# erlgo/openair4G

Measured on AMD Instinct MI355X. Metric: DL subframes/sec (20 MHz, 2x2, 64-QAM), higher is better.
Workload: dtype int16; 1 GPU; dlsim 20 MHz 2x2 TM3 (LARGE_CDD) 64-QAM MCS19x2CW, 2x14 IDFT-2048; config_id=C3, global_batch=8192, subframe_index=7, full_grid=False, parallelism=subframe-sharded x1

## Files before the change

include/oai4g.h:

```cpp
#ifndef OAI4G_H
#define OAI4G_H

#include <stddef.h>
#include <stdint.h>

#ifdef __cplusplus
extern "C" {
#endif

#define OAI4G_LTE_NULL 2
#define OAI4G_NSOFT 1827072
#define OAI4G_MAX_SEGMENTS 16
#define OAI4G_MAX_CHANNEL_BITS (14 * 1200 * 6)
#define OAI4G_D_BYTES (96 + 12 + 3 + 3 * 6144)
#define OAI4G_W_BYTES (3 * 6144 + 96)

enum { OAI4G_SISO = 0, OAI4G_ALAMOUTI = 1, OAI4G_LARGE_CDD = 2 };
enum { OAI4G_CYCLIC_PREFIX = 0, OAI4G_CYCLIC_SUFFIX = 1, OAI4G_ZEROS = 2, OAI4G_NONE = 3 };

typedef struct {
  uint16_t N_RB_DL;
  uint16_t Nid_cell;
  uint8_t Ncp;
  uint8_t nushift;
// ... 57 lines not shown

int oai4g_init(void);
const char *oai4g_last_error(void);
int oai4g_device_name(char *buf, int len);

int oai4g_init_frame_parms(oai4g_frame_parms_t *fp, uint16_t N_RB_DL, uint16_t Nid_cell, uint8_t Ncp,
                           uint8_t nb_antennas_tx, uint8_t mode1_flag, uint8_t frame_type);
uint8_t oai4g_get_Qm(uint8_t mcs);
int oai4g_get_G(const oai4g_frame_parms_t *fp, uint16_t nb_rb, const uint32_t *rb_alloc, uint8_t mod_order,
                uint8_t Nl, uint8_t num_pdcch_symbols, int frame, uint8_t subframe);
uint8_t oai4g_get_Qm_ul(uint8_t mcs);
uint8_t oai4g_get_I_TBS(uint8_t mcs);
uint8_t oai4g_get_I_TBS_UL(uint8_t mcs);
uint32_t oai4g_tbs_bits(uint8_t I_TBS, uint16_t nb_rb);
uint32_t oai4g_get_TBS_DL(uint8_t mcs, uint16_t nb_rb);
uint32_t oai4g_get_TBS_UL(uint8_t mcs, uint16_t nb_rb);
oai4g_dlsch_t *oai4g_new_dlsch(uint8_t Kmimo, uint8_t Mdlharq, uint8_t N_RB_DL);
void oai4g_free_dlsch(oai4g_dlsch_t *dlsch);
uint32_t oai4g_lte_gold_generic(uint32_t *x1, uint32_t *x2, uint8_t reset);
int oai4g_qpp_fold32(uint32_t K, uint32_t *s, uint16_t *tab);
int oai4g_rsc_scan_rows(uint32_t q, uint32_t rows[6]);
int oai4g_rm_pair_schedule(uint32_t C, uint32_t n0, const uint32_t nt[2], const uint32_t wrapt[2],
                           uint32_t *pairs, uint32_t *pair0);

uint32_t oai4g_crc24a(const uint8_t *in, int bitlen);
uint32_t oai4g_crc24b(const uint8_t *in, int bitlen);
int oai4g_lte_segmentation(const uint8_t *input_buffer, uint8_t **output_buffers, uint32_t B, uint32_t *C,
                           uint32_t *Cplus, uint32_t *Cminus, uint32_t *Kplus, uint32_t *Kminus, uint32_t *F);
void oai4g_threegpplte_turbo_encoder(const uint8_t *input, uint16_t input_length_bytes, uint8_t *output,
                                     uint8_t F, uint16_t interleaver_f1, uint16_t interleaver_f2);
uint32_t oai4g_sub_block_interleaving_turbo(uint32_t D, uint8_t *d, uint8_t *w);
uint32_t oai4g_lte_rate_matching_turbo(uint32_t RTC, uint32_t G, const uint8_t *w, uint8_t *e, uint8_t C,
                                       uint32_t Nsoft, uint8_t Mdlharq, uint8_t Kmimo, uint8_t rvidx,
                                       uint8_t Qm, uint8_t Nl, uint8_t r, uint8_t nb_rb, uint8_t m);
int oai4g_dlsch_encoding(uint8_t *a, const oai4g_frame_parms_t *frame_parms, uint8_t num_pdcch_symbols,
                         oai4g_dlsch_t *dlsch, int frame, uint8_t subframe);
void oai4g_dlsch_scrambling(const oai4g_frame_parms_t *frame_parms, int mbsfn_flag, oai4g_dlsch_t *dlsch, int G,
                            uint8_t q, uint8_t Ns);
int oai4g_dlsch_modulation(int32_t **txdataF, int16_t amp, uint32_t subframe_offset,
                           const oai4g_frame_parms_t *frame_parms, uint8_t num_pdcch_symbols,
                           oai4g_dlsch_t *dlsch0, oai4g_dlsch_t *dlsch1);
void oai4g_PHY_ofdm_mod(const int32_t *input, int32_t *output, uint8_t log2fftsize, uint8_t nb_symbols,
                        uint16_t nb_prefix_samples, int etype);
void oai4g_normal_prefix_mod(const int32_t *txdataF, int32_t *txdata, uint8_t nsymb,
                             const oai4g_frame_parms_t *frame_parms);
void oai4g_do_OFDM_mod(int32_t **txdataF, int32_t **txdata, uint32_t frame, uint16_t next_slot,
// ... 208 lines not shown

int oai4g_tx_batch(const oai4g_tx_config_t *cfg, int n_sf, const uint8_t *d_payload, void *d_work,
                   int32_t *d_iq, void *stream);
int oai4g_tx_batch_timed(const oai4g_tx_config_t *cfg, int n_sf, const uint8_t *d_payload, void *d_work,
                         int32_t *d_iq, void *stream, float *kernel_ms);
int oai4g_tx_config_set_control(oai4g_tx_config_t *cfg, uint8_t num_ue_spec_dci, uint8_t num_common_dci,
                                const oai4g_dci_alloc_t *dci_alloc);
#define OAI4G_MAX_PHICH_ITEMS 64
typedef struct {
  uint8_t subframe, ngroup, nseq, hi;
} oai4g_phich_item_t;
typedef struct {
  uint8_t pss_sss;
  uint8_t pbch;
  uint8_t pbch_pdu[3];
  uint8_t frame_mod4;
  uint8_t n_phich;
  oai4g_phich_item_t phich[OAI4G_MAX_PHICH_ITEMS];
} oai4g_common_sig_t;
int oai4g_tx_config_set_common(oai4g_tx_config_t *cfg, const oai4g_common_sig_t *common);
int oai4g_tx_encode(const oai4g_tx_config_t *cfg, int n_sf, const uint8_t *d_payload, void *d_work, void *stream);
int oai4g_tx_modulate(const oai4g_tx_config_t *cfg, int n_sf, const void *d_work, int32_t *d_iq, void *stream);
int oai4g_tx_mod_nosat(const oai4g_tx_config_t *cfg);

int oai4g_diag_encode_phase_ms(const oai4g_tx_config_t *cfg, int n_sf, const uint8_t *d_payload, void *d_work,
                               int stop_phase, int reps, float *ms);
int oai4g_diag_encode_occupancy(const oai4g_tx_config_t *cfg, int *blocks_per_cu, size_t *lds_bytes);
int oai4g_diag_stream(const void *d_src, void *d_dst, size_t bytes, int mode, void *stream);

int oai4g_set_device(int device);
#define OAI4G_DIST_ID_BYTES 128
int oai4g_dist_unique_id(uint8_t id[OAI4G_DIST_ID_BYTES]);
int oai4g_dist_init(int rank, int world, const uint8_t id[OAI4G_DIST_ID_BYTES]);
int oai4g_dist_broadcast_params(oai4g_tx_params_t *p, int root);
int oai4g_dist_allreduce_sum_u64(uint64_t *v, int n);
int oai4g_dist_allreduce_max_f64(double *v, int n);
int oai4g_dist_barrier(void);
int oai4g_dist_rank(void);
int oai4g_dist_world(void);
int oai4g_dist_finalize(void);
void oai4g_shard_range(int n_total, int rank, int world, int *first, int *count);
uint64_t oai4g_payload_seed(uint64_t seed, uint64_t first_subframe, uint32_t n_cw, uint32_t payload_stride);

void *oai4g_dev_alloc(size_t bytes);
void oai4g_dev_free(void *p);
int oai4g_memcpy_h2d(void *dst, const void *src, size_t bytes);
// ... 10 lines not shown
```

openair4g_amd/__init__.py:

```python
import ctypes
import os

import numpy as np

_HERE = os.path.dirname(os.path.abspath(__file__))
LIB_PATH = os.path.join(_HERE, "lib", "libopenair4g_amd.so")

LTE_NULL = 2
NSOFT = 1827072
MAX_SEGMENTS = 16
MAX_CHANNEL_BITS = 14 * 1200 * 6
D_BYTES = 96 + 12 + 3 + 3 * 6144
W_BYTES = 3 * 6144 + 96
SISO, ALAMOUTI, LARGE_CDD = 0, 1, 2
CYCLIC_PREFIX = 0


class OAI4GError(RuntimeError):
    pass


u8p = ctypes.POINTER(ctypes.c_uint8)


# ... 278 lines not shown
    "oai4g_tx_encode": (ctypes.c_int, [ctypes.c_void_p, ctypes.c_int, ctypes.c_void_p, ctypes.c_void_p,
                                       ctypes.c_void_p]),
    "oai4g_tx_modulate": (ctypes.c_int, [ctypes.c_void_p, ctypes.c_int, ctypes.c_void_p, ctypes.c_void_p,
                                         ctypes.c_void_p]),
    "oai4g_tx_mod_nosat": (ctypes.c_int, [ctypes.c_void_p]),
    "oai4g_diag_encode_phase_ms": (ctypes.c_int, [ctypes.c_void_p, ctypes.c_int, ctypes.c_void_p, ctypes.c_void_p,
                                                  ctypes.c_int, ctypes.c_int, ctypes.POINTER(ctypes.c_float)]),
    "oai4g_diag_encode_occupancy": (ctypes.c_int, [ctypes.c_void_p, ctypes.POINTER(ctypes.c_int),
                                                   ctypes.POINTER(ctypes.c_size_t)]),
    "oai4g_diag_stream": (ctypes.c_int, [ctypes.c_void_p, ctypes.c_void_p, ctypes.c_size_t, ctypes.c_int,
                                         ctypes.c_void_p]),
    "oai4g_dev_alloc": (ctypes.c_void_p, [ctypes.c_size_t]),
    "oai4g_dev_free": (None, [ctypes.c_void_p]),
    "oai4g_memcpy_h2d": (ctypes.c_int, [ctypes.c_void_p, ctypes.c_void_p, ctypes.c_size_t]),
    "oai4g_memcpy_d2h": (ctypes.c_int, [ctypes.c_void_p, ctypes.c_void_p, ctypes.c_size_t]),
    "oai4g_memset_d": (ctypes.c_int, [ctypes.c_void_p, ctypes.c_int, ctypes.c_size_t]),
    "oai4g_sync": (ctypes.c_int, []),
    "oai4g_fill_payload": (ctypes.c_int, [ctypes.c_void_p, ctypes.c_size_t, ctypes.c_uint64, ctypes.c_void_p]),
    "oai4g_qpp_fold32": (ctypes.c_int, [ctypes.c_uint32, ctypes.POINTER(ctypes.c_uint32), ctypes.c_void_p]),
    "oai4g_rsc_scan_rows": (ctypes.c_int, [ctypes.c_uint32, ctypes.POINTER(ctypes.c_uint32)]),
    "oai4g_rm_pair_schedule": (ctypes.c_int, [ctypes.c_uint32, ctypes.c_uint32, ctypes.POINTER(ctypes.c_uint32),
                                              ctypes.POINTER(ctypes.c_uint32), ctypes.POINTER(ctypes.c_uint32),
                                              ctypes.POINTER(ctypes.c_uint32)]),
}


def load_library(path=None):
    global _lib
    if _lib is not None:
        return _lib
    path = path or os.environ.get("OAI4G_LIB") or LIB_PATH
    if not os.path.exists(path):
        raise OAI4GError(f"HIP library not built: {path} (run __graft_entry__.build())")
    lib = ctypes.CDLL(path)
    for name, (res, args) in _SIGS.items():
        fn = getattr(lib, name)
        fn.restype = res
        fn.argtypes = args
    _lib = lib
    return lib


def exported_symbols():
    return sorted(_SIGS)


# ... 979 lines not shown
        return ms[0], ms[1]

    def encode_only(self, stream=None):
        _check(self.L.oai4g_tx_encode(self.cfg, self.n_sf, self.d_payload, self.d_work, stream) == 0)

    def diag_encode_phase_ms(self, stop_phase, reps=5):
        ms = ctypes.c_float()
        _check(self.L.oai4g_diag_encode_phase_ms(self.cfg, self.n_sf, self.d_payload, self.d_work, stop_phase, reps,
                                                 ctypes.byref(ms)) == 0)
        return ms.value

    def modulate_only(self, stream=None):
        _check(self.L.oai4g_tx_modulate(self.cfg, self.n_sf, self.d_work, self.d_iq, stream) == 0)

    def upload_ebits(self, words):
        words = np.ascontiguousarray(words, dtype=np.uint32)
        assert words.nbytes <= self.work_bytes
        _check(self.L.oai4g_memcpy_h2d(self.d_work, _ptr(words), words.nbytes) == 0)

    @property
    def mod_nosat(self):
        return bool(self.L.oai4g_tx_mod_nosat(self.cfg))

    def sync(self):
        _check(self.L.oai4g_sync() == 0)

    def ebits(self):
        out = np.empty(self.work_bytes // 4, dtype=np.uint32)
        _check(self.L.oai4g_memcpy_d2h(_ptr(out), self.d_work, out.nbytes) == 0)
        return out.reshape(self.n_sf, self.n_cw, self.ebits_words)

    def iq(self):
        out = np.empty(self.iq_samples, dtype=np.int32)
        _check(self.L.oai4g_memcpy_d2h(_ptr(out), self.d_iq, out.nbytes) == 0)
        return out.reshape(self.n_sf, self.n_ant, self.spt)

    def close(self):
        for p in (self.d_payload, self.d_work, self.d_iq):
            if p:
                self.L.oai4g_dev_free(p)
        self.d_payload = self.d_work = self.d_iq = None
        if self.cfg:
            self.L.oai4g_tx_config_destroy(self.cfg)
            self.cfg = None

    def __del__(self):
# ... 10 lines not shown
```

openair4g_amd/csrc/oai4g_host.cpp:

```cpp
#include <hip/hip_runtime.h>
#include <math.h>
#include <pthread.h>
#include <stdarg.h>
#include <stdio.h>
#include <stdlib.h>
#include <string.h>

#include <algorithm>
#include <cmath>
#include <cstdlib>
#include <vector>
#include <map>
#include <mutex>
#include <vector>

#include "../../include/oai4g.h"
#include "../../include/oai4g_qpp.h"
#include "../../include/oai4g_tbs.h"
#include "oai4g_internal.h"

static thread_local char g_err[512] = "";

static void set_err(const char *fmt, ...)
{
// ... 486 lines not shown
static uint32_t mod_nosat_ok(const cfg_dev_t &h, int v_static)
{
  if (h.log2N != 11 || h.nsymb != 14 || getenv("OAI4G_MOD_SAT")) return 0;
  int v = v_static;
  for (uint32_t cw = 0; cw < h.n_cw; cw++) {
    const cw_dev_t &c = h.cw[cw];
    for (int i = 0; i < 8; i++) v = std::max(v, std::max(std::abs((int)c.qam_a[i]), std::abs((int)c.qam_b[i])));
    v = std::max(v, std::max(std::abs((int)c.qpsk_a), std::abs((int)c.qpsk_b)));
    for (int i = 0; i < 2; i++)
      v = std::max(v, std::max(std::abs((int)c.alm_qpsk[i][0]), std::abs((int)c.alm_qpsk[i][1])));
  }
  const double R = std::sqrt(2.0) * v, band = 12.0 * h.N_RB_DL;
  const double c32 = std::ceil(band / 32) + 1, c8 = std::ceil(band / 8) + 1, c2 = std::ceil(band / 2) + 1;
  return (c32 * R + 128 <= 32767 && c8 * R / 8 + 128 <= 32767 && c2 * R / 16 + 128 <= 32767 &&
          (band + 1) * R / 32 + 128 <= 32767) ? 1u : 0u;
}

static int packed_iq_max(const std::vector<uint32_t> &t)
{
  int v = 0;
  for (uint32_t w : t) v = std::max(v, std::max(std::abs((int)(int16_t)(w & 0xFFFFu)), std::abs((int)(int16_t)(w >> 16))));
  return v;
}

static int not_pilot(int pilots, int re, int nushift, int use2nd)
{
  int off = (pilots == 2) ? 3 : 0, v = nushift % 3;
  if (pilots == 0) return 1;
  if (use2nd) return (re != nushift + off) && (re != ((nushift + 6 + off) % 12));
  return (re != v) && (re != v + 6) && (re != v + 3) && (re != v + 9);
}

static int build_remap(const oai4g_frame_parms_t *fp, const uint32_t *rb_alloc, int num_pdcch, int subframe,
                       int mimo_mode, uint16_t *remap , uint32_t *symbase ,
                       int *re_alloc )
{
  const bool alm = mimo_mode == OAI4G_ALAMOUTI;
  int ralloc = 0;
  int N = fp->ofdm_symbol_size, nsymb = fp->Ncp == 0 ? 14 : 12, half = fp->N_RB_DL >> 1;
  int use2nd = fp->mode1_flag == 1;
  for (int i = 0; i < 14 * N; i++) remap[i] = 0xFFFF;
  uint32_t total = 0;
  for (int l = 0; l < 14; l++) symbase[l] = 0;
  for (int l = num_pdcch; l < nsymb; l++) {
    symbase[l] = total;
    uint32_t idx = 0;
// ... 620 lines not shown
      };
      for (int n = 1; n < 50; n++) step();
      const size_t nw = std::min(stride, (size_t)(h.cw[cw].G[sf] + 31) / 32);
      uint32_t *o = g.data() + ((size_t)sf * h.n_cw + cw) * stride;
      for (size_t w = 0; w < nw; w++) {
        step();
        o[w] = x1 ^ x2;
      }
    }
  if (cfg->d_gold) hipFree(cfg->d_gold);
  cfg->d_gold = nullptr;
  HCK(hipMalloc(&cfg->d_gold, g.size() * 4), -1);
  HCK(hipMemcpy(cfg->d_gold, g.data(), g.size() * 4, hipMemcpyHostToDevice), -1);
  cfg->h.gold_tab = cfg->d_gold;
  return 0;
}

static int upload_cfg(oai4g_tx_config *cfg)
{
  if (upload_remap(cfg) != 0) return -1;
  if (upload_gold(cfg) != 0) return -1;
  cfg->h.with_crs = !cfg->h_crs.empty();
  cfg->h.mod_nosat = mod_nosat_ok(cfg->h, std::max(packed_iq_max(cfg->h_crs), cfg->ctl_vmax));
  cfg->h.n_cu = (uint32_t)g_n_cu;
  cfg->h.gold_x1 = g_gx1;
  cfg->h.gold_x2j = g_gx2j;
  cfg->h.tw = g_tw;
  HCK(hipMalloc(&cfg->d, sizeof(cfg_dev_t)), -1);
  HCK(hipMemcpy(cfg->d, &cfg->h, sizeof(cfg_dev_t), hipMemcpyHostToDevice), -1);
  return 0;
}

static void release_cfg(oai4g_tx_config *cfg)
{
  for (auto &e : cfg->ev_enc)
    if (e) hipEventDestroy(e);
  if (cfg->ev_done) hipEventDestroy(cfg->ev_done);
  if (cfg->s_mod) hipStreamDestroy(cfg->s_mod);
  cfg->s_mod = nullptr;
  cfg->ev_done = nullptr;
  if (cfg->d) hipFree(cfg->d);
  if (cfg->d_remap) hipFree(cfg->d_remap);
  if (cfg->d_stat) hipFree(cfg->d_stat);
  if (cfg->d_gold) hipFree(cfg->d_gold);
  cfg->d_stat = nullptr;
  cfg->d_gold = nullptr;
// ... 106 lines not shown
  for (int i = 0; i < 3; i++) HCK(hipEventCreate(&ev[i]), -1);
  HCK(hipEventRecord(ev[0], s), -1);
  HCK(oai4g_launch_encode(cfg->d, &cfg->h, 0, n_sf, d_payload, (uint32_t *)d_work, s), -1);
  HCK(hipEventRecord(ev[1], s), -1);
  HCK(oai4g_launch_modofdm(cfg->d, &cfg->h, 0, n_sf, (const uint32_t *)d_work, d_iq, s), -1);
  HCK(hipEventRecord(ev[2], s), -1);
  HCK(hipEventSynchronize(ev[2]), -1);
  HCK(hipEventElapsedTime(&kernel_ms[0], ev[0], ev[1]), -1);
  HCK(hipEventElapsedTime(&kernel_ms[1], ev[1], ev[2]), -1);
  for (int i = 0; i < 3; i++) hipEventDestroy(ev[i]);
  return 0;
}

extern "C" int oai4g_tx_modulate(const oai4g_tx_config_t *cfg, int n_sf, const void *d_work, int32_t *d_iq,
                                 void *stream)
{
  NEED_INIT(-1);
  if (!cfg || !iq_aligned(d_iq)) return -1;
  HCK(oai4g_launch_modofdm(cfg->d, &cfg->h, 0, n_sf, (const uint32_t *)d_work, d_iq, (hipStream_t)stream), -1);
  return 0;
}

extern "C" int oai4g_tx_mod_nosat(const oai4g_tx_config_t *cfg) { return cfg ? (int)cfg->h.mod_nosat : 0; }

extern "C" int oai4g_diag_encode_phase_ms(const oai4g_tx_config_t *cfg, int n_sf, const uint8_t *d_payload,
                                          void *d_work, int stop_phase, int reps, float *ms)
{
  NEED_INIT(-1);
  hipEvent_t a, b;
  HCK(hipEventCreate(&a), -1);
  HCK(hipEventCreate(&b), -1);
  HCK(oai4g_launch_encode_phase(cfg->d, &cfg->h, n_sf, d_payload, (uint32_t *)d_work, stop_phase, nullptr), -1);
  HCK(hipEventRecord(a, nullptr), -1);
  for (int i = 0; i < reps; i++)
    HCK(oai4g_launch_encode_phase(cfg->d, &cfg->h, n_sf, d_payload, (uint32_t *)d_work, stop_phase, nullptr), -1);
  HCK(hipEventRecord(b, nullptr), -1);
  HCK(hipEventSynchronize(b), -1);
  HCK(hipEventElapsedTime(ms, a, b), -1);
  *ms /= reps;
  hipEventDestroy(a);
  hipEventDestroy(b);
  return 0;
}

extern "C" int oai4g_diag_encode_occupancy(const oai4g_tx_config_t *cfg, int *blocks_per_cu, size_t *lds_bytes)
{
// ... 1584 lines not shown
      for (uint32_t ant = 0; ant < n_out; ant++) {
        HCK(hipMemcpyAsync(g.data(), dg[ant], gbytes, hipMemcpyDeviceToHost, g_scr.s), -1);
        HCK(hipStreamSynchronize(g_scr.s), -1);
        for (uint32_t l = 0; l < nsymb; l++)
          for (uint32_t k = 0; k < N; k++) {
            const uint32_t v = g[(size_t)l * N + k];
            if (!v) continue;
            tab[(((size_t)sf * 14 + l) * n_tab + ant) * N + k] = v;
            uint16_t &code = cfg->h_remap[((size_t)sf * 14 + l) * N + k];
            if (code != 0xFFFF && code != OAI4G_CTL_CODE) {
              set_err("static REs: subframe %u symbol %u RE %u collides with a PDSCH / CRS RE", sf, l, k);
              return -1;
            }
            code = (uint16_t)OAI4G_CTL_CODE;
            cfg->h.ctlmask[sf] |= 1u << l;
          }
      }
    }
    cfg->h.ctl_on = 1;
    cfg->ctl_vmax = packed_iq_max(tab);
    cfg->h_ctl = std::move(tab);
  }
  cfg->h.mod_nosat = mod_nosat_ok(cfg->h, std::max(packed_iq_max(cfg->h_crs), cfg->ctl_vmax));
  if (upload_remap(cfg) != 0) return -1;
  HCK(hipMemcpy(cfg->d, &cfg->h, sizeof(cfg_dev_t), hipMemcpyHostToDevice), -1);
  return 0;
}

extern "C" int oai4g_tx_config_set_control(oai4g_tx_config_t *cfg, uint8_t n_ue, uint8_t n_common,
                                           const oai4g_dci_alloc_t *dci)
{
  NEED_INIT(-1);
  cfg->dci.assign(dci, dci + ((uint32_t)n_ue + n_common));
  cfg->n_ue_dci = n_ue;
  cfg->n_common_dci = n_common;
  return rebuild_static(cfg);
}

extern "C" int oai4g_tx_config_set_common(oai4g_tx_config_t *cfg, const oai4g_common_sig_t *c)
{
  NEED_INIT(-1);
  if (c && c->n_phich > OAI4G_MAX_PHICH_ITEMS) { set_err("set_common: %u PHICHs", c->n_phich); return -1; }
  if (c && c->n_phich && cfg->p.mode1_flag == 1 && cfg->p.nb_antennas_tx > 1) {
    set_err("set_common: a SISO PHICH on antenna 0 only is not representable in the one-transform TM1 grid");
    return -1;
  }
// ... 1234 lines not shown
```

openair4g_amd/csrc/oai4g_internal.h:

```cpp
#pragma once
#include <hip/hip_runtime.h>
#include <stdint.h>

#include "../../include/oai4g.h"

#define OAI4G_MAX_CB 16
#define OAI4G_MAX_NULLS 104
#define OAI4G_MAX_CHUNKS 192
#define OAI4G_MAX_TASKS (OAI4G_MAX_CB * 20)
#define OAI4G_RM_TILES 20
#define OAI4G_RM_SRC_LAST (1u << 20)
#define OAI4G_RM_DST_WRAP (1u << 27)
#define OAI4G_PIPE_MAX_CHUNKS 16
#define OAI4G_CRS_CODE 0xE000u
#define OAI4G_CTL_CODE 0xC000u
static constexpr uint32_t oai4g_mod_entry_shift(uint32_t mimo_mode, uint32_t n_ant, uint32_t log2N)
{
  return log2N != 11 ? 1u : mimo_mode == OAI4G_LARGE_CDD && n_ant == 2 ? 3u : mimo_mode == OAI4G_SISO ? 2u : 1u;
}
static constexpr uint32_t oai4g_mod_addr_mask(uint32_t shift) { return 0x7FFFu & ~((1u << shift) - 1u); }
static constexpr uint32_t oai4g_mod_sentinel(uint32_t N) { return (3u * N) / 4u; }
static constexpr bool oai4g_mod_nre_fits(uint32_t nre, uint32_t N) { return nre + 3u <= oai4g_mod_sentinel(N); }
#define OAI4G_ENC_CRC_TABLE_WORDS (256 + 256)
#define OAI4G_GOLD_LANES 256
#define OAI4G_GOLD_STRIDE 17
#define OAI4G_MAX_GOLD_WORDS (OAI4G_GOLD_LANES * OAI4G_GOLD_STRIDE)
#define OAI4G_TW_TOTAL (16 + 64 + 128 + 256 + 512 + 1024 + 2048)

static inline __host__ __device__ uint32_t oai4g_tw_offset(int log2s)
{
  switch (log2s) {
  case 4: return 0;
  case 6: return 16;
  case 7: return 80;
  case 8: return 208;
  case 9: return 464;
  case 10: return 976;
  case 11: return 2000;
  default: return 0;
  }
}

struct cw_dev_t {
  uint32_t TBS;
  uint32_t A_bytes;
// ... 38 lines not shown
  uint32_t crc_lpb;
  uint32_t crcmul_tb[8][6][16];
  uint32_t crcmul_blk[OAI4G_MAX_CB][96];
  uint32_t crc2_tb[2][8][96];
  uint32_t crc2_cb[2][2][8][96];
  uint32_t rm_src[2][OAI4G_RM_TILES + 1][32];
  uint32_t rm_dst[2][OAI4G_RM_TILES + 1][32];
  uint32_t rm_pair0[OAI4G_MAX_CB + 1];
  uint32_t rm_pairs[OAI4G_MAX_CB * ((OAI4G_RM_TILES + 1) / 2)];
};

struct cfg_dev_t {
  uint32_t N_RB_DL, N, log2N, cp0, cp, spt, nsymb, n_ant, first_carrier;
  uint32_t n_cw, mimo_mode, num_pdcch, rnti, Nid_cell, first_sf, sf_step;
  uint32_t payload_stride;
  uint32_t ebits_words;
  uint32_t lds_tb_words;
  uint32_t lds_stream_words;
  uint32_t lds_gold_words;
  uint32_t lds_w_words;
  uint32_t lds_a_words;
  uint32_t lds_b_words;
  uint32_t mod_nosat;
  uint32_t pad;
  uint32_t crctab[2][256];
  cw_dev_t cw[2];
  uint32_t symbase[10][14];
  uint32_t symnre[10][14];
  uint32_t n_cu;
  const uint16_t *remap;
  const uint16_t *remap_tm;
  uint32_t with_crs;
  uint32_t pilmask;
  uint32_t ctlmask[10];
  uint32_t ctl_on;
  const uint32_t *gold_tab;
  const uint32_t *gold_x1;
  const uint32_t *gold_x2j;
  const uint32_t *tw;
  const uint32_t *stat_tm;
  uint32_t stat_planes;
  uint32_t pad2;
};

hipError_t oai4g_launch_encode(const cfg_dev_t *d_cfg, const cfg_dev_t *h_cfg, int sf0, int n_sf,
                               const uint8_t *d_payload, uint32_t *d_ebits, hipStream_t s);
hipError_t oai4g_encode_occupancy(const cfg_dev_t *h_cfg, int *blocks_per_cu, size_t *lds_bytes);
// ... 35 lines not shown
                            size_t out_stride, uint8_t *d_iters, uint32_t max_it, uint32_t crc_type, uint32_t F,
                            const uint16_t *d_pi, uint8_t *d_scratch, hipStream_t s);
#define OAI4G_UL_MAX_C 16
struct ul_pat_t {
  uint32_t D, R, Ncb, Nnn, k0c;
  uint32_t k0cr[4];
  const uint8_t *dummy;
  const uint32_t *cidx;
};
struct ul_dev_t {
  uint32_t C, Rmax;
  uint32_t E[OAI4G_UL_MAX_C], off[OAI4G_UL_MAX_C], pat_of[OAI4G_UL_MAX_C];
  ul_pat_t pat[3];
};
hipError_t oai4g_launch_ul_rm_deint(const ul_dev_t *d_cfg, const ul_dev_t *h_cfg, int n_tb, const int16_t *d_e,
                                    size_t e_stride, int16_t *d_dfull, size_t d_stride, hipStream_t s);
hipError_t oai4g_launch_ul_rm_harq(const ul_dev_t *d_cfg, const ul_dev_t *h_cfg, int n_tb, const int16_t *d_e,
                                   size_t e_stride, int16_t *d_w, size_t w_stride, uint32_t rv, int clear,
                                   int16_t *d_dfull, size_t d_stride, hipStream_t s);
hipError_t oai4g_launch_rm_rx(const int16_t *d_soft, uint32_t E, int16_t *d_w, const uint8_t *d_dummy,
                              const uint32_t *d_cidx, uint32_t Ncb, uint32_t Nnn, uint32_t k0c, int clear, hipStream_t s);
hipError_t oai4g_launch_subblock_deint(uint32_t D, int16_t *d_dfull, const int16_t *d_w, hipStream_t s);

hipError_t oai4g_launch_modofdm(const cfg_dev_t *d_cfg, const cfg_dev_t *h_cfg, int sf0, int n_sf,
                                const uint32_t *d_ebits, int32_t *d_iq, hipStream_t s);
struct ofdm_sym_t {
  uint32_t in_off;
  uint32_t out_off;
  uint32_t cp;
};
hipError_t oai4g_launch_ofdm(const int32_t *d_in, int32_t *d_out, int log2n, int nsym, const ofdm_sym_t *syms,
                             int scale, const uint32_t *d_tw, hipStream_t s);
hipError_t oai4g_launch_idft_strided(const int32_t *d_in, int32_t *d_out, int log2n, int n_jobs, size_t in_stride,
                                     uint32_t in_off, size_t out_stride, int scale, const uint32_t *d_tw, hipStream_t s);
hipError_t oai4g_launch_freq_offset(const int32_t *d_est, size_t est_stride, int n_jobs, int N_RB, uint32_t row_off,
                                    uint32_t prev_off, int32_t *d_omega, hipStream_t s);
struct pcfich_args_t {
  uint32_t c_init;
  uint32_t cfi;
  int16_t gain;
  uint8_t mode1;
  uint8_t nushift3;
  uint32_t reg_off[4];
  uint32_t n_ant;
};
hipError_t oai4g_launch_pcfich(int32_t *d_g0, int32_t *d_g1, const pcfich_args_t &a, hipStream_t s);
// ... 135 lines not shown
```

openair4g_amd/csrc/oai4g_ofdm.hip:

```cpp
#include "oai4g_internal.h"

#include "oai4g_dft_prims.h"

__host__ __device__ constexpr int tw_distinct(int T, int SC, int J) { return T >= SC ? 1 : (SC / T < J ? SC / T : J); }

template <int LOG2N>
struct idft_tw_t {
  static constexpr int N = 1 << LOG2N, T = N >> 4;
  static constexpr bool HAS256 = LOG2N >= 8, HAS1024 = LOG2N >= 10, HASR2 = (LOG2N & 1) != 0;
  static constexpr int D64 = tw_distinct(T, 16, 4), D256 = tw_distinct(T, 64, 4), D1024 = tw_distinct(T, 256, 4),
                       DR2 = tw_distinct(T, N / 2, 8);
  twp_t l16[7];
  s16x2 l64[D64][3];
  s16x2 l256[HAS256 ? D256 : 1][3];
  s16x2 l1024[HAS1024 ? D1024 : 1][3];
  s16x2 r2[HASR2 ? DR2 : 1];

  __device__ __forceinline__ void load(const uint32_t *tw, int t)
  {
    gu32_t *g = (gu32_t *)tw;
    constexpr int i16[7] = {0, 1, 2, 3, 4, 6, 9};
#pragma unroll
    for (int i = 0; i < 7; i++)
      l16[i] = {u2c(g[oai4g_tw_offset(4) + i16[i]]), u2c(g[OAI4G_TW_TOTAL + oai4g_tw_offset(4) + i16[i]])};
// ... 670 lines not shown
  constexpr uint32_t IPS = MODE == 3 ? 2u : 1u;
  __shared__ __attribute__((aligned(16))) uint32_t lds_data[UNITS * NA * LDSW];
  constexpr bool SEARLY = CRS && (NA == 1 || LOG2N < 11);
  constexpr int SW = G::SW, SENT = G::SENT, QPT = G::QPT, QROW = G::QROW;
  constexpr uint32_t QZERO = 4u * 4u * QROW;
  constexpr bool ALIAS = LOG2N == 11;
  static_assert(!ALIAS || (UNITS == 1 && 2 * SW <= 2 * NA * LDSW), "staged addresses must fit the exchange");
  __shared__ __attribute__((aligned(16))) uint16_t lds_s_own[ALIAS ? 1 : UNITS][2][SW];
  uint16_t(*lds_s)[2][SW] = ALIAS ? (uint16_t(*)[2][SW])lds_data : lds_s_own;
  __shared__ uint32_t qtab[4 * QROW + 1];
  constexpr uint32_t ESH = oai4g_mod_entry_shift(MODE == 0 ? OAI4G_SISO : MODE == 1 ? OAI4G_ALAMOUTI : OAI4G_LARGE_CDD,
                                                 MODE == 3 ? 4 : 2, LOG2N);
  constexpr uint32_t EMASK = oai4g_mod_addr_mask(ESH);
  constexpr bool PRE = ESH == 3;
  static_assert(!PRE || (MODE == 2 && ALIAS && SW * 8 <= NA * LDSW * 4), "the precoded pairs must fit the exchange");
  u32x2_t *lds_p = (u32x2_t *)lds_data;
  constexpr bool PRE1 = ESH == 2;
  static_assert(!PRE1 || (MODE == 0 && ALIAS && SW * 4 <= NA * LDSW * 4), "the staged QAM words must fit the exchange");
  uint32_t *lds_w = (uint32_t *)lds_data;
  const int unit = threadIdx.x / T, t = threadIdx.x % T;
  typename idft_sel<LOG2N>::tw_t twr;
  twr.load(c->tw, t);
  const uint32_t n_ant = c->n_ant;
  constexpr uint32_t nsymb = ECP ? 12u : 14u;
  constexpr uint32_t sps = ECP ? 6 : 7;
  for (uint32_t i = threadIdx.x; i < 4 * QROW + 1; i += blockDim.x) {
    const uint32_t row = i / QROW, bits = i - row * QROW, cw = row >> 1, pil = row & 1;
    uint32_t v = 0;
    if (row < 4) {
      if constexpr (MODE == 1) {
        const cw_dev_t &w = c->cw[0];
        v = c2u(cw ? alm_tb(bits, w, pil) : alm_ta(bits, w, pil));
      } else {
        const cw_dev_t &w = c->cw[cw];
        v = c2u(qam_map(bits, w.Qm, pil ? w.qam_b : w.qam_a, pil ? w.qpsk_b : w.qpsk_a));
      }
    }
    qtab[i] = v;
  }
  if (!ALIAS)
    for (uint32_t i = threadIdx.x; i < UNITS * 4; i += blockDim.x) lds_s[i >> 2][(i >> 1) & 1][SENT + (i & 1)] = QZERO;
  const uint32_t Qm0 = c->cw[0].Qm, Qm1 = c->cw[1].Qm;
  const uint32_t mask0 = (1u << Qm0) - 1u, mask1 = (1u << Qm1) - 1u;
  const uint32_t qt0 = 4u * Qm0 * (uint32_t)t, qt1 = 4u * Qm1 * (uint32_t)t;
  __syncthreads();

  const int stride = __builtin_amdgcn_readfirstlane(gridDim.x * UNITS);
  struct pf_t {
    u32x4_t ra, rb;
    uint32_t x0[QPT], x1[QPT];
  } pf;
  typedef const __attribute__((address_space(4))) cfg_dev_t ccfg_t;
  const ccfg_t *cc = (const ccfg_t *)c;
  auto fetch = [&](int bse) {
    const int item = bse + (UNITS == 1 ? 0 : unit);
    const bool act = item < n_items;
    const uint32_t it0 = (act ? (uint32_t)item : 0u) / IPS;
    const uint32_t it = UNITS == 1 ? __builtin_amdgcn_readfirstlane(it0) : it0;
    const uint32_t sf = it / nsymb, l = it - sf * nsymb;
    const uint32_t sfi = (cc->first_sf + (sf0 + sf) * cc->sf_step) % 10;
    const uint32_t nre_u = cc->symnre[sfi][l], re0 = cc->symbase[sfi][l];
    const uint32_t nre = act ? nre_u : 0u;
    const gu128_t *rsrc = (const gu128_t *)(cc->remap_tm + ((size_t)sfi * 14 + l) * N + (size_t)t * 16);
    pf.ra = rsrc[0];
    pf.rb = rsrc[1];
    if (act && nre) {
      const uint8_t *esf = (const uint8_t *)(ebits + (size_t)(sf * cc->n_cw) * cc->ebits_words);
      const uint32_t nq = (nre + 3) >> 2;
      const uint32_t b0 = re0 * Qm0, lim0 = 4 * Qm0 * (nq - 1), b1 = re0 * Qm1, lim1 = 4 * Qm1 * (nq - 1);
#pragma unroll
      for (int k = 0; k < QPT; k++) {
        pf.x0[k] = ld_u32_any(esf + ((b0 + min(qt0 + (uint32_t)(4 * T * k) * Qm0, lim0)) >> 3));
        if constexpr (CW2)
          pf.x1[k] = ld_u32_any(esf + (size_t)4 * cc->ebits_words + ((b1 + min(qt1 + (uint32_t)(4 * T * k) * Qm1, lim1)) >> 3));
      }
    }
  };
  fetch(blockIdx.x * UNITS);
  __builtin_amdgcn_s_waitcnt(0x0F70);

  for (int base = blockIdx.x * UNITS; base < n_items; base += stride) {
    const int item = base + (UNITS == 1 ? 0 : unit);
    const bool active = item < n_items;
    const uint32_t it0 = (active ? (uint32_t)item : 0u) / IPS, pair = (uint32_t)item % IPS;
    const uint32_t it = UNITS == 1 ? __builtin_amdgcn_readfirstlane(it0) : it0;
    const uint32_t sf = it / nsymb, l = it - sf * nsymb;
    const uint32_t sfi = (cc->first_sf + (sf0 + sf) * cc->sf_step) % 10;
    const uint32_t nre_u = cc->symnre[sfi][l], re0 = cc->symbase[sfi][l];
    const uint32_t nre = active ? nre_u : 0u;
    const bool crs_sym = (cc->pilmask >> l) & 1u;
    const bool stat_sym = (cc->with_crs && crs_sym) || ((cc->ctlmask[sfi] >> l) & 1u);
    const uint32_t pil = crs_sym ? 1u : 0u;
    const uint32_t slot = l >= sps ? 1u : 0u, si = l - slot * sps;
    const uint32_t body = slot * (cc->spt >> 1) + (si == 0 ? cc->cp0 : (N + cc->cp0) + (si - 1) * (N + cc->cp) + cc->cp);
    const int cp = (int)(si == 0 ? cc->cp0 : cc->cp);
    uint32_t *dst0 = (uint32_t *)iq + (size_t)sf * n_ant * cc->spt + body;

    if (UNITS == 1 && nre == 0 && !(CRS && stat_sym)) {
      fetch(base + stride);
      __builtin_amdgcn_s_waitcnt(0x0F70);
      if (active)
        for (uint32_t a = MODE == 3 ? 2 * pair : 0; a < (MODE == 3 ? 2 * pair + 2 : n_ant); a++) {
          uint32_t *d = dst0 + (size_t)a * cc->spt - cp;
          for (int f = t; f < N + cp; f += T) d[f] = 0u;
        }
      continue;
    }

    const uint32_t rw[8] = {pf.ra.x, pf.ra.y, pf.ra.z, pf.ra.w, pf.rb.x, pf.rb.y, pf.rb.z, pf.rb.w};
    if constexpr (OAI4G_MOD_PRIO >= 1) __builtin_amdgcn_s_setprio(OAI4G_MOD_PRIO == 3 ? 3 : 2);
    if (PRE) {
      if (active && t < 2) lds_p[SENT + t] = (u32x2_t){0u, 0u};
    } else if (PRE1) {
      if (active && t < 2) lds_w[SENT + t] = 0u;
    } else if (ALIAS && active && t < 4) lds_s[0][t >> 1][SENT + (t & 1)] = QZERO;
    if (active && nre) {
      const uint32_t nq = (nre + 3) >> 2;
      const uint32_t sh0 = (re0 * Qm0 + qt0) & 7u, sh1 = (re0 * Qm1 + qt1) & 7u;
      const uint32_t m40 = mask0 << 2, m41 = mask1 << 2;
// ... 228 lines not shown
          }
        },
        1, it);
    if (PSYNC) __syncthreads();
  }
}

template <int LOG2N, int MODE, bool CRS, bool ECP, bool NS = false>
static hipError_t launch_modofdm_t(const cfg_dev_t *d_cfg, const cfg_dev_t *h_cfg, int sf0, int n_items,
                                   const uint32_t *d_ebits, int32_t *d_iq, hipStream_t s)
{
  static int occ = 0;
  if (!occ) {
    if (hipOccupancyMaxActiveBlocksPerMultiprocessor(&occ, k_modofdm<LOG2N, MODE, CRS, ECP, NS>, 128, 0) != hipSuccess ||
        occ < 1)
      occ = 1;
    if (const char *e = getenv("OAI4G_MODOFDM_OCC")) {
      const int cap = atoi(e);
      if (cap >= 1 && cap < occ) occ = cap;
    }
  }
  const int units = modofdm_geom<LOG2N>::UNITS;
  int want = (n_items + units - 1) / units, cap = occ * (int)h_cfg->n_cu;
  int grid = want < cap ? want : cap;
  if (grid < 1) grid = 1;
  hipLaunchKernelGGL((k_modofdm<LOG2N, MODE, CRS, ECP, NS>), dim3(grid), dim3(128), 0, s, d_cfg, n_items, d_ebits, d_iq,
                     (uint32_t)sf0);
  return hipGetLastError();
}

template <int LOG2N, int MODE, bool ECP>
static hipError_t launch_modofdm_c(const cfg_dev_t *d_cfg, const cfg_dev_t *h_cfg, int sf0, int n_items,
                                   const uint32_t *d_ebits, int32_t *d_iq, hipStream_t s)
{
  if (h_cfg->with_crs || h_cfg->ctl_on) {
    if constexpr (LOG2N == 11 && !ECP)
      if (h_cfg->mod_nosat) return launch_modofdm_t<LOG2N, MODE, true, ECP, true>(d_cfg, h_cfg, sf0, n_items, d_ebits, d_iq, s);
    return launch_modofdm_t<LOG2N, MODE, true, ECP>(d_cfg, h_cfg, sf0, n_items, d_ebits, d_iq, s);
  }
  if constexpr (LOG2N == 11 && !ECP)
    if (h_cfg->mod_nosat) return launch_modofdm_t<LOG2N, MODE, false, ECP, true>(d_cfg, h_cfg, sf0, n_items, d_ebits, d_iq, s);
  return launch_modofdm_t<LOG2N, MODE, false, ECP>(d_cfg, h_cfg, sf0, n_items, d_ebits, d_iq, s);
}

template <int LOG2N, bool ECP>
static hipError_t launch_modofdm_m(const cfg_dev_t *d_cfg, const cfg_dev_t *h_cfg, int sf0, int n_items,
// ... 1 lines not shown
{
  switch (h_cfg->mimo_mode) {
  case OAI4G_LARGE_CDD:
    return h_cfg->n_ant == 4 ? launch_modofdm_c<LOG2N, 3, ECP>(d_cfg, h_cfg, sf0, 2 * n_items, d_ebits, d_iq, s)
                             : launch_modofdm_c<LOG2N, 2, ECP>(d_cfg, h_cfg, sf0, n_items, d_ebits, d_iq, s);
  case OAI4G_ALAMOUTI: return launch_modofdm_c<LOG2N, 1, ECP>(d_cfg, h_cfg, sf0, n_items, d_ebits, d_iq, s);
  default: return launch_modofdm_c<LOG2N, 0, ECP>(d_cfg, h_cfg, sf0, n_items, d_ebits, d_iq, s);
  }
}

template <int LOG2N>
static hipError_t launch_modofdm_n(const cfg_dev_t *d_cfg, const cfg_dev_t *h_cfg, int sf0, int n_items,
                                   const uint32_t *d_ebits, int32_t *d_iq, hipStream_t s)
{
  return h_cfg->nsymb == 12 ? launch_modofdm_m<LOG2N, true>(d_cfg, h_cfg, sf0, n_items, d_ebits, d_iq, s)
                            : launch_modofdm_m<LOG2N, false>(d_cfg, h_cfg, sf0, n_items, d_ebits, d_iq, s);
}

hipError_t oai4g_launch_modofdm(const cfg_dev_t *d_cfg, const cfg_dev_t *h_cfg, int sf0, int n_sf,
                                const uint32_t *d_ebits, int32_t *d_iq, hipStream_t s)
{
  if (n_sf <= 0) return hipSuccess;
  if (h_cfg->nsymb != 12 && h_cfg->nsymb != 14) return hipErrorInvalidValue;
  const int n_items = n_sf * (int)h_cfg->nsymb;
  d_ebits += (size_t)sf0 * h_cfg->n_cw * h_cfg->ebits_words;
  d_iq += (size_t)sf0 * h_cfg->n_ant * h_cfg->spt;
  if (h_cfg->mimo_mode != OAI4G_SISO && h_cfg->n_ant != 2 && !(h_cfg->mimo_mode == OAI4G_LARGE_CDD && h_cfg->n_ant == 4))
    return hipErrorInvalidValue;
  if (h_cfg->mimo_mode == OAI4G_LARGE_CDD && h_cfg->n_cw != 2) return hipErrorInvalidValue;
  if (h_cfg->log2N >= 7 && h_cfg->log2N <= 11) {
    const uint32_t T = h_cfg->N >> 4, zlo = h_cfg->log2N == 8 ? 6u : 5u, zhi = h_cfg->log2N == 8 ? 9u : 10u;
    if (h_cfg->first_carrier != h_cfg->N - 6 * h_cfg->N_RB_DL || T * zlo <= 6 * h_cfg->N_RB_DL ||
        T * (zhi + 1) > h_cfg->first_carrier)
      return hipErrorInvalidValue;
  }
  switch (h_cfg->log2N) {
  case 7: return launch_modofdm_n<7>(d_cfg, h_cfg, sf0, n_items, d_ebits, d_iq, s);
  case 8: return launch_modofdm_n<8>(d_cfg, h_cfg, sf0, n_items, d_ebits, d_iq, s);
  case 9: return launch_modofdm_n<9>(d_cfg, h_cfg, sf0, n_items, d_ebits, d_iq, s);
  case 10: return launch_modofdm_n<10>(d_cfg, h_cfg, sf0, n_items, d_ebits, d_iq, s);
  case 11: return launch_modofdm_n<11>(d_cfg, h_cfg, sf0, n_items, d_ebits, d_iq, s);
  default: return hipErrorInvalidValue;
  }
}

__global__ void __launch_bounds__(256) k_modulate_bytes(const cfg_dev_t *__restrict__ c, int sfi,
                                                        const uint8_t *__restrict__ e0,
// ... 83 lines not shown
```

Measured before the change: 8.951 million subframes/s.

## Skip leading empty OFDM symbols in modofdm, zero-filling them from first active symbol

When neither CRS nor control channels are present, the host finds how many leading symbols of every subframe carry no REs. The modulation/IDFT kernel then only schedules the remaining symbols per subframe, and the first scheduled symbol writes zeros over the preceding time-domain samples. Item-to-(subframe, symbol) mapping now uses a precomputed magic-multiply reciprocal instead of division. An optional grid cap hook is also added. This removes IDFT work for empty symbols at the cost of an extra zero-fill loop and more validation logic.

```diff
diff --git a/include/oai4g.h b/include/oai4g.h
--- a/include/oai4g.h
+++ b/include/oai4g.h
@@ -103,6 +103,9 @@
 int oai4g_rsc_scan_rows(uint32_t q, uint32_t rows[6]);
 int oai4g_rm_pair_schedule(uint32_t C, uint32_t n0, const uint32_t nt[2], const uint32_t wrapt[2],
                            uint32_t *pairs, uint32_t *pair0);
+int oai4g_mod_item_map(uint32_t item, uint32_t ips, uint32_t lz, uint32_t per, uint32_t *sf, uint32_t *l,
+                       uint32_t *pair);
+void oai4g_set_modofdm_grid_cap(int n_workgroups);
 
 uint32_t oai4g_crc24a(const uint8_t *in, int bitlen);
 uint32_t oai4g_crc24b(const uint8_t *in, int bitlen);
@@ -357,6 +360,7 @@
 int oai4g_tx_encode(const oai4g_tx_config_t *cfg, int n_sf, const uint8_t *d_payload, void *d_work, void *stream);
 int oai4g_tx_modulate(const oai4g_tx_config_t *cfg, int n_sf, const void *d_work, int32_t *d_iq, void *stream);
 int oai4g_tx_mod_nosat(const oai4g_tx_config_t *cfg);
+int oai4g_tx_mod_lz(const oai4g_tx_config_t *cfg);
 
 int oai4g_diag_encode_phase_ms(const oai4g_tx_config_t *cfg, int n_sf, const uint8_t *d_payload, void *d_work,
                                int stop_phase, int reps, float *ms);
diff --git a/openair4g_amd/__init__.py b/openair4g_amd/__init__.py
--- a/openair4g_amd/__init__.py
+++ b/openair4g_amd/__init__.py
@@ -324,6 +324,11 @@
     "oai4g_rm_pair_schedule": (ctypes.c_int, [ctypes.c_uint32, ctypes.c_uint32, ctypes.POINTER(ctypes.c_uint32),
                                               ctypes.POINTER(ctypes.c_uint32), ctypes.POINTER(ctypes.c_uint32),
                                               ctypes.POINTER(ctypes.c_uint32)]),
+    "oai4g_mod_item_map": (ctypes.c_int, [ctypes.c_uint32, ctypes.c_uint32, ctypes.c_uint32, ctypes.c_uint32,
+                                          ctypes.POINTER(ctypes.c_uint32), ctypes.POINTER(ctypes.c_uint32),
+                                          ctypes.POINTER(ctypes.c_uint32)]),
+    "oai4g_set_modofdm_grid_cap": (None, [ctypes.c_int]),
+    "oai4g_tx_mod_lz": (ctypes.c_int, [ctypes.c_void_p]),
 }
 
 
@@ -1349,6 +1354,10 @@
     def mod_nosat(self):
         return bool(self.L.oai4g_tx_mod_nosat(self.cfg))
 
+    @property
+    def mod_lz(self):
+        return self.L.oai4g_tx_mod_lz(self.cfg)
+
     def sync(self):
         _check(self.L.oai4g_sync() == 0)
 
diff --git a/openair4g_amd/csrc/oai4g_host.cpp b/openair4g_amd/csrc/oai4g_host.cpp
--- a/openair4g_amd/csrc/oai4g_host.cpp
+++ b/openair4g_amd/csrc/oai4g_host.cpp
@@ -532,6 +532,34 @@
   for (uint32_t w : t) v = std::max(v, std::max(std::abs((int)(int16_t)(w & 0xFFFFu)), std::abs((int)(int16_t)(w >> 16))));
   return v;
 }
+
+static void mod_items_setup(cfg_dev_t &h)
+{
+  uint32_t lz = 0;
+  if (!h.with_crs && !h.ctl_on)
+    for (; lz < OAI4G_MOD_LZ_MAX && lz + 1 < h.nsymb / 2; lz++) {
+      bool empty = true;
+      for (int sf = 0; sf < 10 && empty; sf++) empty = h.symnre[sf][lz] == 0;
+      if (!empty) break;
+    }
+  h.mod_lz = lz;
+  h.mod_per = h.nsymb - lz;
+  h.mod_permag = oai4g_mod_permag(h.mod_per);
+}
+
+extern "C" int oai4g_mod_item_map(uint32_t item, uint32_t ips, uint32_t lz, uint32_t per, uint32_t *sf, uint32_t *l,
+                                  uint32_t *pair)
+{
+  if (ips < 1 || ips > 2 || per < 1 || lz > OAI4G_MOD_LZ_MAX) return -1;
+  const oai4g_mod_item_t m = oai4g_mod_item(item, ips, lz, per, oai4g_mod_permag(per));
+  *sf = m.sf;
+  *l = m.l;
+  *pair = m.pair;
+  return m.l == lz && lz > 0 ? 1 : 0;
+}
+
+int g_modofdm_grid_cap = 0;
+extern "C" void oai4g_set_modofdm_grid_cap(int n_workgroups) { g_modofdm_grid_cap = n_workgroups > 0 ? n_workgroups : 0; }
 
 static int not_pilot(int pilots, int re, int nushift, int use2nd)
 {
@@ -1198,6 +1226,7 @@
   if (upload_gold(cfg) != 0) return -1;
   cfg->h.with_crs = !cfg->h_crs.empty();
   cfg->h.mod_nosat = mod_nosat_ok(cfg->h, std::max(packed_iq_max(cfg->h_crs), cfg->ctl_vmax));
+  mod_items_setup(cfg->h);
   cfg->h.n_cu = (uint32_t)g_n_cu;
   cfg->h.gold_x1 = g_gx1;
   cfg->h.gold_x2j = g_gx2j;
@@ -1350,6 +1379,7 @@
 }
 
 extern "C" int oai4g_tx_mod_nosat(const oai4g_tx_config_t *cfg) { return cfg ? (int)cfg->h.mod_nosat : 0; }
+extern "C" int oai4g_tx_mod_lz(const oai4g_tx_config_t *cfg) { return cfg ? (int)cfg->h.mod_lz : -1; }
 
 extern "C" int oai4g_diag_encode_phase_ms(const oai4g_tx_config_t *cfg, int n_sf, const uint8_t *d_payload,
                                           void *d_work, int stop_phase, int reps, float *ms)
@@ -2980,6 +3010,7 @@
     cfg->h_ctl = std::move(tab);
   }
   cfg->h.mod_nosat = mod_nosat_ok(cfg->h, std::max(packed_iq_max(cfg->h_crs), cfg->ctl_vmax));
+  mod_items_setup(cfg->h);
   if (upload_remap(cfg) != 0) return -1;
   HCK(hipMemcpy(cfg->d, &cfg->h, sizeof(cfg_dev_t), hipMemcpyHostToDevice), -1);
   return 0;
diff --git a/openair4g_amd/csrc/oai4g_internal.h b/openair4g_amd/csrc/oai4g_internal.h
--- a/openair4g_amd/csrc/oai4g_internal.h
+++ b/openair4g_amd/csrc/oai4g_internal.h
@@ -21,6 +21,18 @@
 static constexpr uint32_t oai4g_mod_addr_mask(uint32_t shift) { return 0x7FFFu & ~((1u << shift) - 1u); }
 static constexpr uint32_t oai4g_mod_sentinel(uint32_t N) { return (3u * N) / 4u; }
 static constexpr bool oai4g_mod_nre_fits(uint32_t nre, uint32_t N) { return nre + 3u <= oai4g_mod_sentinel(N); }
+struct oai4g_mod_item_t {
+  uint32_t sf, l, pair;
+};
+static constexpr uint32_t oai4g_mod_permag(uint32_t per) { return (uint32_t)(((1ull << 32) + per - 1) / per); }
+static inline __host__ __device__ oai4g_mod_item_t oai4g_mod_item(uint32_t item, uint32_t ips, uint32_t lz, uint32_t per,
+                                                                  uint32_t permag)
+{
+  const uint32_t it = item / ips;
+  const uint32_t sf = (uint32_t)(((uint64_t)it * permag) >> 32);
+  return {sf, lz + it - sf * per, item - it * ips};
+}
+#define OAI4G_MOD_LZ_MAX 4u
 #define OAI4G_ENC_CRC_TABLE_WORDS (256 + 256)
 #define OAI4G_GOLD_LANES 256
 #define OAI4G_GOLD_STRIDE 17
@@ -105,7 +117,7 @@
   uint32_t lds_a_words;
   uint32_t lds_b_words;
   uint32_t mod_nosat;
-  uint32_t pad;
+  uint32_t mod_lz, mod_per, mod_permag;
   uint32_t crctab[2][256];
   cw_dev_t cw[2];
   uint32_t symbase[10][14];
@@ -187,6 +199,7 @@
                               const uint32_t *d_cidx, uint32_t Ncb, uint32_t Nnn, uint32_t k0c, int clear, hipStream_t s);
 hipError_t oai4g_launch_subblock_deint(uint32_t D, int16_t *d_dfull, const int16_t *d_w, hipStream_t s);
 
+extern int g_modofdm_grid_cap;
 hipError_t oai4g_launch_modofdm(const cfg_dev_t *d_cfg, const cfg_dev_t *h_cfg, int sf0, int n_sf,
                                 const uint32_t *d_ebits, int32_t *d_iq, hipStream_t s);
 struct ofdm_sym_t {
diff --git a/openair4g_amd/csrc/oai4g_ofdm.hip b/openair4g_amd/csrc/oai4g_ofdm.hip
--- a/openair4g_amd/csrc/oai4g_ofdm.hip
+++ b/openair4g_amd/csrc/oai4g_ofdm.hip
@@ -716,7 +716,6 @@
   typename idft_sel<LOG2N>::tw_t twr;
   twr.load(c->tw, t);
   const uint32_t n_ant = c->n_ant;
-  constexpr uint32_t nsymb = ECP ? 12u : 14u;
   constexpr uint32_t sps = ECP ? 6 : 7;
   for (uint32_t i = threadIdx.x; i < 4 * QROW + 1; i += blockDim.x) {
     const uint32_t row = i / QROW, bits = i - row * QROW, cw = row >> 1, pil = row & 1;
@@ -746,12 +745,15 @@
   } pf;
   typedef const __attribute__((address_space(4))) cfg_dev_t ccfg_t;
   const ccfg_t *cc = (const ccfg_t *)c;
+  constexpr uint32_t nsymb = ECP ? 12u : 14u;
+  const uint32_t lz = CRS ? 0u : cc->mod_lz, per = CRS ? nsymb : cc->mod_per;
+  const uint32_t permag = CRS ? oai4g_mod_permag(nsymb) : cc->mod_permag;
   auto fetch = [&](int bse) {
     const int item = bse + (UNITS == 1 ? 0 : unit);
     const bool act = item < n_items;
-    const uint32_t it0 = (act ? (uint32_t)item : 0u) / IPS;
-    const uint32_t it = UNITS == 1 ? __builtin_amdgcn_readfirstlane(it0) : it0;
-    const uint32_t sf = it / nsymb, l = it - sf * nsymb;
+    const uint32_t it0 = act ? (uint32_t)item : 0u;
+    const oai4g_mod_item_t m = oai4g_mod_item(UNITS == 1 ? __builtin_amdgcn_readfirstlane(it0) : it0, IPS, lz, per, permag);
+    const uint32_t sf = m.sf, l = m.l;
     const uint32_t sfi = (cc->first_sf + (sf0 + sf) * cc->sf_step) % 10;
     const uint32_t nre_u = cc->symnre[sfi][l], re0 = cc->symbase[sfi][l];
     const uint32_t nre = act ? nre_u : 0u;
@@ -776,9 +778,10 @@
   for (int base = blockIdx.x * UNITS; base < n_items; base += stride) {
     const int item = base + (UNITS == 1 ? 0 : unit);
     const bool active = item < n_items;
-    const uint32_t it0 = (active ? (uint32_t)item : 0u) / IPS, pair = (uint32_t)item % IPS;
+    const uint32_t it0 = active ? (uint32_t)item : 0u;
     const uint32_t it = UNITS == 1 ? __builtin_amdgcn_readfirstlane(it0) : it0;
-    const uint32_t sf = it / nsymb, l = it - sf * nsymb;
+    const oai4g_mod_item_t m = oai4g_mod_item(it, IPS, lz, per, permag);
+    const uint32_t sf = m.sf, l = m.l, pair = m.pair;
     const uint32_t sfi = (cc->first_sf + (sf0 + sf) * cc->sf_step) % 10;
     const uint32_t nre_u = cc->symnre[sfi][l], re0 = cc->symbase[sfi][l];
     const uint32_t nre = active ? nre_u : 0u;
@@ -789,6 +792,15 @@
     const uint32_t body = slot * (cc->spt >> 1) + (si == 0 ? cc->cp0 : (N + cc->cp0) + (si - 1) * (N + cc->cp) + cc->cp);
     const int cp = (int)(si == 0 ? cc->cp0 : cc->cp);
     uint32_t *dst0 = (uint32_t *)iq + (size_t)sf * n_ant * cc->spt + body;
+
+    if (lz && l == lz && active) {
+      const uint32_t fl = body - (uint32_t)cp;
+      for (uint32_t a = MODE == 3 ? 2 * pair : 0; a < (MODE == 3 ? 2 * pair + 2 : n_ant); a++) {
+        uint32_t *d = (uint32_t *)iq + ((size_t)sf * n_ant + a) * cc->spt;
+        for (uint32_t f = t; f < fl / 2; f += T) ((u32x2_t *)d)[f] = (u32x2_t){0u, 0u};
+        if ((fl & 1u) && t == 0) d[fl - 1] = 0u;
+      }
+    }
 
     if (UNITS == 1 && nre == 0 && !(CRS && stat_sym)) {
       fetch(base + stride);
@@ -1063,6 +1075,7 @@
   }
   const int units = modofdm_geom<LOG2N>::UNITS;
   int want = (n_items + units - 1) / units, cap = occ * (int)h_cfg->n_cu;
+  if (g_modofdm_grid_cap > 0 && g_modofdm_grid_cap < cap) cap = g_modofdm_grid_cap;
   int grid = want < cap ? want : cap;
   if (grid < 1) grid = 1;
   hipLaunchKernelGGL((k_modofdm<LOG2N, MODE, CRS, ECP, NS>), dim3(grid), dim3(128), 0, s, d_cfg, n_items, d_ebits, d_iq,
@@ -1110,7 +1123,11 @@
 {
   if (n_sf <= 0) return hipSuccess;
   if (h_cfg->nsymb != 12 && h_cfg->nsymb != 14) return hipErrorInvalidValue;
-  const int n_items = n_sf * (int)h_cfg->nsymb;
+  const uint32_t lz = h_cfg->mod_lz, per = h_cfg->mod_per;
+  if (lz > OAI4G_MOD_LZ_MAX || lz >= h_cfg->nsymb / 2 || per != h_cfg->nsymb - lz || h_cfg->mod_permag != oai4g_mod_permag(per) ||
+      (uint64_t)n_sf * per * per > (1ull << 30) || (lz && ((h_cfg->spt & 1u) || h_cfg->with_crs || h_cfg->ctl_on)))
+    return hipErrorInvalidValue;
+  const int n_items = n_sf * (int)per;
   d_ebits += (size_t)sf0 * h_cfg->n_cw * h_cfg->ebits_words;
   d_iq += (size_t)sf0 * h_cfg->n_ant * h_cfg->spt;
   if (h_cfg->mimo_mode != OAI4G_SISO && h_cfg->n_ant != 2 && !(h_cfg->mimo_mode == OAI4G_LARGE_CDD && h_cfg->n_ant == 4))
```

Result: faster. 9.186 million subframes/s (median of 6 runs) (+2.6%).
